# BogdanDIA/gr-dvbt

Measured on AMD Instinct MI355X. Metric: RX Msamples/s (baseband in -> TS out), higher is better.
Workload: dtype u8 (Viterbi/RS) + f32 (front end)

## Files before the change

gr_dvbt_amd/csrc/k_viterbi3.hpp:

```cpp
#pragma once
#include <hip/hip_runtime.h>
#include <stdint.h>
#include <limits.h>
#include <string.h>
#include "dvbt_tables.hpp"
#include "k_backend.hpp"

namespace dvbt {

inline VitParams make_vit_params(const Dims &d, int bsize, int chunk_bytes)
{
  VitParams v; memset(&v, 0, sizeof v);
  v.m = d.m; v.k = d.k; v.n = d.n; v.plen = d.plen; v.ntb = d.ntb; v.bsize = bsize;
  v.d_nsymbols = bsize * d.n / d.m; v.d_nbits = 2 * d.k * bsize;
  v.chunk_bytes = chunk_bytes > 0 ? chunk_bytes : 768; v.payload = d.payload; v.warm = 72;
  memcpy(v.punct, d.punct, 16); memcpy(v.prefix, d.prefix, 16);
  v.punct_mask = 0; v.prefix_nib = 0;
  for (int i = 0; i < d.plen; i++) { v.punct_mask |= (unsigned)d.punct[i] << i; v.prefix_nib |= (unsigned long long)d.prefix[i] << (4 * i); }
  v.magic_plen = ~0ull / (unsigned)d.plen + 1; v.magic_m = ~0ull / (unsigned)d.m + 1;
  for (int i = 0; i < 64; i++) v.punct_rep |= (unsigned long long)d.punct[i % d.plen] << i;
  v.magic16_plen = (65536u + (unsigned)d.plen - 1) / (unsigned)d.plen;
  return v;
}

// ... 23 lines not shown
typedef short v3pk __attribute__((ext_vector_type(2)));
__device__ __forceinline__ v3pk pk(int x) { return __builtin_bit_cast(v3pk, x); }
__device__ __forceinline__ int ipk(v3pk x) { return __builtin_bit_cast(int, x); }
__device__ __forceinline__ int pk_add(int a, int b) { return ipk(pk(a) + pk(b)); }
__device__ __forceinline__ int pk_sub(int a, int b) { return ipk(pk(a) - pk(b)); }
__device__ __forceinline__ int pk_max(int a, int b) { return ipk(__builtin_elementwise_max(pk(a), pk(b))); }
__device__ __forceinline__ int pk_min(int a, int b) { return ipk(__builtin_elementwise_min(pk(a), pk(b))); }
template <int CTRL> __device__ __forceinline__ int dppb(int v) { return __builtin_amdgcn_update_dpp(0, v, CTRL, 0xf, 0xf, true); }
__device__ __forceinline__ int vconst(int c) { int x; asm("v_mov_b32 %0, %1" : "=v"(x) : "s"(c)); return x; }
__device__ __forceinline__ int pk_max_swap(int a, int b) { int r; asm("v_pk_max_i16 %0, %1, %2 op_sel:[0,1] op_sel_hi:[1,0]" : "=v"(r) : "v"(a), "v"(b)); return r; }

struct V3Lane {
  unsigned sel[6][2];
  int bias8[6][2];
  int kc[3][2];
  int org[2];
  int arm_mid[3][2];
  int arm_b2[3][2];
  int arm_org[3][2];
};

__device__ __forceinline__ int v3_phys(int a) { const int a2 = (a >> 2) & 1; return (a & 8) | (a2 << 2) | ((a & 3) ^ (a2 ? 3 : 0)); }
__device__ __forceinline__ int v3_log(int p) { const int q = p & 7, a2 = (q >> 2) & 1; return (p & 8) | (a2 << 2) | ((q ^ (a2 ? 7 : 0)) & 3); }
__device__ __forceinline__ int v3_cell_of_z(int z) { return ((z & 2) << 4) | ((z & 1) << 4) | v3_log(z >> 2); }
__device__ __forceinline__ int v3_z_of_cell(int c) { return v3_phys(c & 15) * 4 + ((c >> 5) & 1) * 2 + ((c >> 4) & 1); }

__device__ __forceinline__ int v3_upper(int P, int r, int h, int a) { const int c = (r << 5) | (h << 4) | a; return (c >> (5 - P)) & 1; }
__device__ inline void v3_init_lane(int pl, V3Lane &L)
{
  const int a = v3_log(pl);
  for (int r = 0; r < 2; r++) {
    for (int P = 0; P < 6; P++) {
      unsigned idx[2];
      for (int h = 0; h < 2; h++) {
        const int c = (r << 5) | (h << 4) | a, i = rotl6(c, P) & 31;
        const int c0 = ((i >> 2) ^ (i >> 1) ^ i) & 1;
        const int c1 = ((i >> 4) ^ (i >> 2) ^ (i >> 1)) & 1;
        idx[h] = (unsigned)(c0 | (c1 << 1));
      }
      L.sel[P][r] = 0x0c | (idx[0] << 8) | (0x0cu << 16) | (idx[1] << 24);
      L.bias8[P][r] = (v3_upper(P, r, 0, a) << 8) | (v3_upper(P, r, 1, a) << 24);
    }
    L.org[r] = (pl * 4 + 2 * r) | ((pl * 4 + 2 * r + 1) << 16);
    for (int e = 0; e < 3; e++) {
      const int P0 = 2 * e;
      const int s0 = rotl6((r << 5) | a, P0), s1 = rotl6((r << 5) | 16 | a, P0);
      L.kc[e][r] = ((63 - s0) | ((63 - s1) << 16)) | (L.bias8[P0][r] ^ 0x01000100);
      const int b2 = ((s0 >> 4) << 6) | (((s1 >> 4) << 6) << 16);
      L.arm_mid[e][r] = (L.bias8[(P0 + 3) % 6][r] >> 2) | (L.bias8[(P0 + 4) % 6][r] >> 1) | L.bias8[(P0 + 5) % 6][r];
      L.arm_org[e][r] = L.org[r] | (L.bias8[P0][r] >> 2) | (L.bias8[P0 + 1][r] >> 1) | L.bias8[(P0 + 2) % 6][r];
      L.arm_b2[e][r] = b2 | L.bias8[P0][r];
    }
  }
}

template <int P, int ST> __device__ __forceinline__ void v3_step(int (&v)[2], unsigned W, const V3Lane &L, int (&raw)[2])
{
  int X[2], Y[2], mx[2];
  const int D0 = (int)__builtin_amdgcn_perm(0u, W, L.sel[P][0]);
  X[0] = pk_add(v[0], D0); Y[0] = pk_sub(v[0], D0);
  if (P == 0 || P == 4) { X[1] = pk_add(v[1], D0); Y[1] = pk_sub(v[1], D0); }
  else if (P == 2 || P == 3) { X[1] = pk_sub(v[1], D0); Y[1] = pk_add(v[1], D0); }
  else {
    const int D1 = (int)__builtin_amdgcn_perm(0u, W, L.sel[P][1]);
    X[1] = pk_add(v[1], D1); Y[1] = pk_sub(v[1], D1);
  }
  if (P == 0) { mx[0] = pk_max(X[0], Y[1]); mx[1] = pk_max(X[1], Y[0]); }
  else if (P == 1) { mx[0] = pk_max_swap(X[0], Y[0]); mx[1] = pk_max_swap(X[1], Y[1]); }
  else {
#pragma unroll
    for (int r = 0; r < 2; r++)
      mx[r] = pk_max(X[r], P == 2 ? dppb<DPP_ROR8>(Y[r]) : P == 3 ? dppb<DPP_HALF_MIRROR>(Y[r]) : P == 4 ? dppb<DPP_XOR2>(Y[r]) : dppb<DPP_XOR1>(Y[r]));
  }
  constexpr int PN = (P + 1) % 6;
#pragma unroll
  for (int r = 0; r < 2; r++) {
    if (ST == 0) v[r] = mx[r];
    else if (ST == 3) v[r] = (mx[r] & (int)0xfe3ffe3f) | L.arm_mid[((PN + 3) % 6) / 2][r];
    else if (ST == 1) v[r] = (mx[r] & (int)0xfe3ffe3f) | L.arm_b2[PN / 2][r];
    else if (ST == 4) v[r] = (mx[r] & (int)0xfefffeff) | L.bias8[PN][r];
    else { raw[r] = mx[r]; v[r] = (mx[r] & (int)0xfe00fe00) | L.arm_org[PN / 2][r]; }
  }
}

#if V3_EXP & 64
#define V3_YIELD() asm volatile("s_nop 3" ::: "memory")
#else
#define V3_YIELD()
#endif
template <int P0> __device__ __forceinline__ void v3_window(int (&v)[2], const unsigned (&W)[8], const V3Lane &L, int (&raw)[2])
{
  v3_step<(P0 + 0) % 6, 0>(v, W[0], L, raw); V3_YIELD(); v3_step<(P0 + 1) % 6, 0>(v, W[1], L, raw); V3_YIELD(); v3_step<(P0 + 2) % 6, 3>(v, W[2], L, raw); V3_YIELD();
  v3_step<(P0 + 3) % 6, 0>(v, W[3], L, raw); V3_YIELD(); v3_step<(P0 + 4) % 6, 0>(v, W[4], L, raw); V3_YIELD(); v3_step<(P0 + 5) % 6, 1>(v, W[5], L, raw); V3_YIELD();
  v3_step<(P0 + 6) % 6, 4>(v, W[6], L, raw); V3_YIELD(); v3_step<(P0 + 7) % 6, 2>(v, W[7], L, raw);
}

__device__ __forceinline__ int lo16(int x) { return (x << 16) >> 16; }
__device__ __forceinline__ int hi16(int x) { return x >> 16; }
template <int CTRL> __device__ __forceinline__ int max_dpp(int v) { return max(v, dppb<CTRL>(v)); }
template <int CTRL> __device__ __forceinline__ int min_dpp(int v) { return min(v, dppb<CTRL>(v)); }

template <int PE, bool RENORM> __device__ __forceinline__ int v3_window_end(int (&v)[2], const V3Lane &L)
{
  const int kp = pk_max((v[0] & (int)0xfe00fe00) | L.kc[PE / 2][0], (v[1] & (int)0xfe00fe00) | L.kc[PE / 2][1]);
  int k = max(lo16(kp), hi16(kp));
  k = max_dpp<DPP_XOR1>(k); k = max_dpp<DPP_XOR2>(k); k = max_dpp<DPP_HALF_MIRROR>(k); k = max_dpp<DPP_MIRROR>(k);
  if (RENORM) {
    const unsigned sub = (unsigned)((k & ~0x1ff) - (48 << 8));
    const int mn = (int)__builtin_amdgcn_perm(sub, sub, 0x01000100u);
    v[0] = pk_sub(v[0], mn); v[1] = pk_sub(v[1], mn);
  }
  return k;
}

struct V3Trace {
  int z[2];
  int wsh[2];
  int wlast[2];
  bool ok[2];
  long long ob[2];
};
__device__ __forceinline__ void v3_hop(V3Trace &T, const unsigned char *tab, int rowc)
{
#pragma unroll
  for (int q = 0; q < 2; q++) {
    const unsigned t = tab[T.z[q]];
    T.wsh[q] -= 256;
    T.z[q] = (T.wsh[q] & 0x3fc0) | ((int)t & ~0x3fc0);
  }
}
__device__ __forceinline__ void v3_trace_out(const V3Trace &T, const unsigned char *tab, int rowc, uint8_t *out, long long out_lo)
{
#pragma unroll
  for (int q = 0; q < 2; q++) {
    const unsigned t = tab[T.z[q]];
    const int w = T.wlast[q];
    const int sstart = rotl6(v3_cell_of_z((int)(t & 63u)), 2 * (((w % 3) + 3) % 3));
    if (T.ok[q]) out[T.ob[q] - out_lo] = (unsigned char)((sstart << 2) | (t >> 6));
  }
}

template <int V6, bool HOPS, int HOP0, int NTB> __device__ __forceinline__ void v3_fwd_window(int (&v)[2], const V3Lane &L, const unsigned *wrow, unsigned char *tab,
                                                                                           unsigned char *bests, int j0, int dd, int pl, V3Trace &T)
{
  if (HOPS && HOP0 + 2 * V6 < NTB - 1) v3_hop(T, tab, dd * 64);
  if (HOPS && HOP0 + 2 * V6 + 1 < NTB - 1) v3_hop(T, tab, dd * 64);
  const int jr = (j0 + V6) & (V3_RINGW - 1);
  unsigned W[8];
#if V3_EXP & 256
  for (int i = 0; i < 8; i++) { W[i] = (unsigned)(j0 * 0x01010101 + i * 0x00020406 + pl); asm volatile("" : "+v"(W[i])); }
#else
  {
    const uint4 *wp = reinterpret_cast<const uint4 *>(wrow + V6 * 8);
    const uint4 t0 = wp[0], t1 = wp[1];
    W[0] = t0.x; W[1] = t0.y; W[2] = t0.z; W[3] = t0.w; W[4] = t1.x; W[5] = t1.y; W[6] = t1.z; W[7] = t1.w;
  }
#endif
  constexpr int P0 = (8 * V6) % 6;
  int raw[2];
#if V3_EXP & 32
  if (V6 & 1) __builtin_amdgcn_s_setprio(1); else __builtin_amdgcn_s_setprio(0);
#endif
#if V3_EXP & 128
  __builtin_amdgcn_s_sleep(1);
#endif
  v3_window<P0>(v, W, L, raw);
  if (!(V3_EXP & 4)) *reinterpret_cast<unsigned *>(tab + (jr * 4 + dd) * 64 + pl * 4) = __builtin_amdgcn_perm((unsigned)raw[1], (unsigned)raw[0], 0x06040200u);
  if (V3_EXP & 2) { if (raw[0] == 0x12345) bests[jr] = 1; return; }
  const int s = v3_window_end<(P0 + 2) % 6, (V6 & 1) == 1>(v, L);
  bests[dd * V3_RINGW + jr] = (unsigned char)s;
}
template <bool HOPS, int HOP0, int NTB> __device__ __forceinline__ void v3_fwd_six(int (&v)[2], const V3Lane &L, const unsigned *wrow, unsigned char *tab,
                                                                                  unsigned char *bests, int j0, int dd, int pl, V3Trace &T)
{
  v3_fwd_window<0, HOPS, HOP0, NTB>(v, L, wrow, tab, bests, j0, dd, pl, T); v3_fwd_window<1, HOPS, HOP0, NTB>(v, L, wrow, tab, bests, j0, dd, pl, T);
  v3_fwd_window<2, HOPS, HOP0, NTB>(v, L, wrow, tab, bests, j0, dd, pl, T); v3_fwd_window<3, HOPS, HOP0, NTB>(v, L, wrow, tab, bests, j0, dd, pl, T);
  v3_fwd_window<4, HOPS, HOP0, NTB>(v, L, wrow, tab, bests, j0, dd, pl, T); v3_fwd_window<5, HOPS, HOP0, NTB>(v, L, wrow, tab, bests, j0, dd, pl, T);
}

#if V3_EXP & 16
__device__ unsigned long long *v3_dbg;
#endif

constexpr int V3_SLOT = 32;
constexpr int V3_CTL_CHUNKS = 0;
constexpr int V3_CTL_MISMATCH = 1;
constexpr int V3_CTL_CONFLICT = 2;
constexpr int V3_CTL_UNPROVEN = 3;
constexpr int V3_CTL_SEQ = 4;
constexpr int V3_CTL_ACC = 8;
constexpr int V3_CTL_HDR = 16;
struct V3Aux {
  int *snap;
  int *ctl;
  long long cap;
  long long grid0;
  const int *carry_in;
  int *carry_out; int carry_rel;
  int debug;
};
__device__ __forceinline__ int *v3_own(const V3Aux &ax, long long c) { return ax.snap + (3 * c) * V3_SLOT; }
__device__ __forceinline__ int *v3_pred(const V3Aux &ax, long long c) { return ax.snap + (3 * c + 1) * V3_SLOT; }
__device__ __forceinline__ int *v3_fix(const V3Aux &ax, long long c) { return ax.snap + (3 * c + 2) * V3_SLOT; }
inline size_t v3_snap_words(long long cap) { return (size_t)(cap + 2) * 3 * V3_SLOT; }
inline size_t v3_ctl_words(long long cap) { return (size_t)V3_CTL_HDR + 2 * (size_t)(cap + 2); }

struct V3Lds { unsigned char *tab; unsigned *wbuf; unsigned char *bests; const unsigned *lut; };
__device__ __forceinline__ void v3_init_lut(unsigned *lut, int lane)
{
  if (lane < 16) {
    const int k0 = (lane >> 2) & 1, k1 = (lane >> 3) & 1, t1 = (lane >> 1) & 1, t0 = lane & 1;
    const int u0 = k0 ? 1 - 2 * t1 : 0, u1 = k1 ? 1 - 2 * (k0 ? t0 : t1) : 0;
    const unsigned d0 = (unsigned)(2 * (u0 + u1)) & 0xff, d1 = (unsigned)(2 * (-u0 + u1)) & 0xff;
    const unsigned d2 = (unsigned)(2 * (u0 - u1)) & 0xff, d3 = (unsigned)(2 * (-u0 - u1)) & 0xff;
    lut[lane] = d0 | (d1 << 8) | (d2 << 16) | (d3 << 24);
  }
}

template <int NTB, int WARM, int MODE>
__device__ __forceinline__ void v3_decode(const uint8_t *__restrict__ in, uint8_t *__restrict__ out, long long total_steps, long long total_out, const VitParams &vp,
                                          long long in_base, long long out_lo, long long b0, bool dec_active, const V3Lds &S, const V3Lane &L, int (&v)[2], int (&endv)[2],
                                          int *own, int *predn, const int *inject, int *carry, int carry_rel)
{
  unsigned char *const tab = S.tab; unsigned *const wbuf = S.wbuf; unsigned char *const bests = S.bests; const unsigned *const lut = S.lut;
  unsigned *const cbits = wbuf;
  constexpr int V3_CBS = V3_BLK * 8;
  static_assert(V3_CBW <= V3_CBS, "bit stream does not fit the step-word row");
  const int lane = threadIdx.x & 63, dd = lane >> 4, pl = lane & 15;
  const int B = vp.chunk_bytes, m = vp.m;
  constexpr int ntb = NTB;
  const long long b1 = (b0 + B < total_out) ? b0 + B : total_out;
  const int warm = MODE == 2 ? 0 : WARM > 0 ? WARM : vp.warm;
  const long long w0 = b0 + 2 - warm;
  const int J = ((warm + B + ntb - 1 + V3_BLK - 1) / V3_BLK) * V3_BLK;
  const long long n_in_bytes = (total_steps * 2 / vp.plen * vp.n + vp.m - 1) / vp.m;
  const int nload = ((384 + 2 * m - 2) / m + 3 + 15) / 16;

  int ph0 = 0, bo0 = 0, off = 0; uint4 q = make_uint4(0, 0, 0, 0);
  auto stage_load = [&](int jb) {
    const long long tb = 8 * (w0 - 1) + (long long)jb * 8 - 2;
    const unsigned long long pbit = 2ull * (unsigned long long)(tb > 0 ? tb : 0);
    const unsigned long long pq = __umul64hi(pbit, vp.magic_plen);
    ph0 = (int)(pbit - pq * (unsigned)vp.plen);
    const unsigned long long rb = pq * (unsigned)vp.n + ((vp.prefix_nib >> (4 * ph0)) & 15ull);
    const unsigned long long by = __umul64hi(rb, vp.magic_m);
    const long long byte0 = (long long)by; bo0 = (int)(rb - by * (unsigned)m);
    off = (int)(((unsigned long long)(uintptr_t)in + (unsigned long long)(byte0 - in_base)) & 3ull);
    const long long src = byte0 - off + pl * 16;
    q = make_uint4(0, 0, 0, 0);
    if (dec_active && pl < nload) {
      if (src >= in_base && src + 16 <= n_in_bytes) q = *reinterpret_cast<const uint4 *>(in + (src - in_base));
      else {
        unsigned w[4] = {0, 0, 0, 0};
        for (int i = 0; i < 16; i++) {
          const long long bb = src + i;
          const unsigned bv = (bb >= in_base && bb < n_in_bytes) ? in[bb - in_base] : 0;
          w[i >> 2] |= bv << (8 * (i & 3));
        }
        q = make_uint4(w[0], w[1], w[2], w[3]);
      }
    }
  };
  auto stage_words = [&](int jb) {
    {
      const unsigned mk = (1u << m) - 1;
      auto grp = [&](unsigned d) { return ((d & mk) << (3 * m)) | (((d >> 8) & mk) << (2 * m)) | (((d >> 16) & mk) << m) | ((d >> 24) & mk); };
      const unsigned g0 = grp(q.x), g1 = grp(q.y), g2 = grp(q.z), g3 = grp(q.w);
      unsigned *cb = cbits + dd * V3_CBS;
      if (pl < nload) {
        if (m == 2) cb[pl] = (g0 << 24) | (g1 << 16) | (g2 << 8) | g3;
        else if (m == 4) { cb[2 * pl] = (g0 << 16) | g1; cb[2 * pl + 1] = (g2 << 16) | g3; }
        else { cb[3 * pl] = (g0 << 8) | (g1 >> 16); cb[3 * pl + 1] = (g1 << 16) | (g2 >> 8); cb[3 * pl + 2] = (g2 << 24) | g3; }
      }
    }
    __builtin_amdgcn_fence(__ATOMIC_SEQ_CST, "wavefront");
    constexpr int SPL = V3_BLK * 8 / 16;
    const long long tb = 8 * (w0 - 1) + (long long)jb * 8 - 2;
    const long long tbr = tb > 0 ? tb : 0;
    const int ub0 = pl * SPL;
    const long long t = tb + ub0;
    int lo = 0;
    if (t < 0) lo = (-t < SPL) ? (int)(-t) : SPL;
    const long long rem = total_steps - t;
    int hi = !dec_active ? 0 : rem <= 0 ? 0 : rem < SPL ? (int)rem : SPL;
    if (hi < lo) hi = lo;
    int x = ph0 + 2 * (int)((t + lo) - tbr);
    if (x < 0) x = 0;
    const int dq = (int)(((unsigned)x * vp.magic16_plen) >> 16);
    const int ph = x - dq * vp.plen;
    const int pos = off * m + bo0 + dq * vp.n + (int)((vp.prefix_nib >> (4 * ph)) & 15ull) - (int)((vp.prefix_nib >> (4 * ph0)) & 15ull);
    const unsigned kmask = ((unsigned)(vp.punct_rep >> ph) << (2 * lo)) & (((1u << (2 * hi)) - 1u) & ~((1u << (2 * lo)) - 1u));
    const unsigned *cb = cbits + dd * V3_CBS;
    const unsigned cw0 = cb[pos >> 5], cw1 = cb[(pos >> 5) + 1];
    unsigned win = (unsigned)(((((unsigned long long)cw0) << 32) | cw1) >> (32 - (pos & 31)));
#pragma unroll
    for (int i = 0; i < SPL; i++) {
      const unsigned k2 = (kmask >> (2 * i)) & 3u;
      const unsigned idx = (k2 << 2) | (win >> 30);
      win <<= (k2 - (k2 >> 1));
      wbuf[dd * (V3_BLK * 8) + ub0 + i] = lut[idx];
    }
    __builtin_amdgcn_fence(__ATOMIC_SEQ_CST, "wavefront");
  };
  V3Trace T;
  auto trace_init = [&](int jp) {
#pragma unroll
    for (int c = 0; c < 2; c++) {
      int jj = jp + c * 16 + pl;
      T.ob[c] = b0 + (jj - (warm + ntb - 1));
      T.ok[c] = (c * 16 + pl < V3_BLK) && dec_active && jj >= warm + ntb - 1 && T.ob[c] < b1 && (MODE != 1 || T.ob[c] >= out_lo);
      if (!T.ok[c]) jj = jp;
      const int sb = 63 - (bests[dd * V3_RINGW + (jj & (V3_RINGW - 1))] & 63);
      T.wsh[c] = ((jj << 8) & 0x3f00) | (dd * 64);
      T.z[c] = v3_z_of_cell(((sb | (sb << 6)) >> ((8 * jj + 8) % 6)) & 63) | T.wsh[c];
      T.wlast[c] = jj - (ntb - 1);
    }
  };

  stage_load(0);
  for (int jb = 0; jb < J; jb += V3_BLK) {
    if (MODE == 1 && dec_active) {
      if (jb == warm) { if (inject) { v[0] = inject[0]; v[1] = inject[1]; } own[0] = v[0]; own[1] = v[1]; }
      if (jb == warm + B) { predn[0] = v[0]; predn[1] = v[1]; }
      if (carry && jb == warm + carry_rel) { carry[0] = v[0]; carry[1] = v[1]; }
    }
    if (MODE == 2) {
      if (jb == 0 && dec_active) { own[0] = v[0]; own[1] = v[1]; }
      if (jb == B) { endv[0] = v[0]; endv[1] = v[1]; }
      if (carry && dec_active && jb == carry_rel) { carry[0] = v[0]; carry[1] = v[1]; }
    }
    if (!(V3_EXP & 8) || jb == 0) stage_words(jb);
    if (jb + V3_BLK < J && !(V3_EXP & 8)) stage_load(jb + V3_BLK);
    const bool tr = jb > 0 && !(V3_EXP & 1);
    if (tr) trace_init(jb - V3_BLK);
    const unsigned *wrow = wbuf + dd * (V3_BLK * 8);
    if (tr) {
      v3_fwd_six<true, 0, NTB>(v, L, wrow, tab, bests, jb, dd, pl, T);
      v3_fwd_six<true, 12, NTB>(v, L, wrow + 48, tab, bests, jb + 6, dd, pl, T);
      v3_trace_out(T, tab, dd * 64, out, out_lo);
    } else {
      v3_fwd_six<false, 0, NTB>(v, L, wrow, tab, bests, jb, dd, pl, T);
      v3_fwd_six<false, 0, NTB>(v, L, wrow + 48, tab, bests, jb + 6, dd, pl, T);
    }
    for (int wi = 12; wi < V3_BLK; wi += 6) v3_fwd_six<false, 0, NTB>(v, L, wrow + wi * 8, tab, bests, jb + wi, dd, pl, T);
  }
  __builtin_amdgcn_fence(__ATOMIC_SEQ_CST, "wavefront");
  trace_init(J - V3_BLK);
  for (int h = 0; h < ntb - 1; h++) v3_hop(T, tab, dd * 64);
  v3_trace_out(T, tab, dd * 64, out, out_lo);
}

#define V3_LDS_DECL(NW) \
  __shared__ __attribute__((aligned(16))) unsigned char tab_[NW][V3_RINGW * 4 * 64];    \
  __shared__ __attribute__((aligned(16))) unsigned wbuf_[NW][4 * V3_BLK * 8];           \
  __shared__ unsigned char bests_[NW][4 * V3_RINGW];                                     \
  __shared__ unsigned lut[16];

template <int NTB, int WARM = V3_WARM, int MODE = 0> __global__ __launch_bounds__(64 * V3_WGW) void viterbi3_kernel(const uint8_t *__restrict__ in, uint8_t *__restrict__ out, const RxState *st,
                                                      long long steps_fixed, VitParams vp, V3Aux ax, long long in_base, long long out_lo)
{
  V3_LDS_DECL(V3_WGW)
  const int wv = V3_WGW > 1 ? (int)(threadIdx.x >> 6) : 0;
  const V3Lds S = {tab_[wv], wbuf_[wv], bests_[wv], lut};
  const int lane = threadIdx.x & 63, dd = lane >> 4, pl = lane & 15;
  const long long total_steps = st ? st->n_vit_steps : steps_fixed;
  const long long total_out = total_steps / 8 - vp.ntb;
  const int B = vp.chunk_bytes;
  if (MODE == 1 && blockIdx.x == 0 && threadIdx.x == 0) {
    ax.ctl[V3_CTL_MISMATCH] = 0; ax.ctl[V3_CTL_CONFLICT] = 0; ax.ctl[V3_CTL_UNPROVEN] = -1; ax.ctl[V3_CTL_SEQ] = 0;
  }
  const long long grid0 = MODE == 1 ? ax.grid0 : out_lo;
  const long long chunk0 = ((long long)blockIdx.x * V3_WGW + wv) * 4;
  if (grid0 + chunk0 * B >= total_out) return;
  const long long c = chunk0 + dd, b0 = grid0 + c * B;
  const bool dec_active = b0 < total_out;
  v3_init_lut(lut, lane);
#if V3_EXP & 16
  const unsigned long long dbg_t0 = wall_clock64();
#endif
  V3Lane L; v3_init_lane(pl, L);
  int v[2] = {L.arm_org[0][0], L.arm_org[0][1]}, endv[2];
  int *own = nullptr, *predn = nullptr, *carry = nullptr; const int *inject = nullptr;
  if (MODE == 1) {
    own = v3_own(ax, c) + 2 * pl; predn = v3_pred(ax, c + 1) + 2 * pl;
    if (c == 0 && ax.carry_in) inject = ax.carry_in + 2 * pl;
    if (ax.carry_out && b0 + B >= total_out) carry = ax.carry_out + 2 * pl;
  }
  v3_decode<NTB, WARM, MODE>(in, out, total_steps, total_out, vp, in_base, out_lo, b0, dec_active, S, L, v, endv, own, predn, inject, carry, ax.carry_rel);
#if V3_EXP & 16
  if (lane == 0) {
    unsigned id, xcc;
    asm volatile("s_getreg_b32 %0, hwreg(HW_REG_HW_ID)" : "=s"(id));
    asm volatile("s_getreg_b32 %0, hwreg(HW_REG_XCC_ID)" : "=s"(xcc));
    unsigned long long *d = v3_dbg + 3 * ((long long)blockIdx.x * V3_WGW + wv);
    d[0] = (id & 0xffffu) | ((xcc & 0xfu) << 16); d[1] = dbg_t0; d[2] = wall_clock64();
  }
#endif
}

__device__ __forceinline__ long long v3_nchunks(long long total_out, long long grid0, int B) { return total_out > grid0 ? (total_out - grid0 + B - 1) / B : 0; }
__device__ __forceinline__ bool v3_slots_equal(const int *a_, const int *b_)
{
  const int4 *a = reinterpret_cast<const int4 *>(a_), *b = reinterpret_cast<const int4 *>(b_);
  bool same = true;
#pragma unroll
  for (int i = 0; i < 8; i++) { const int4 x = a[i], y = b[i]; same = same && x.x == y.x && x.y == y.y && x.z == y.z && x.w == y.w; }
  return same;
}

__global__ __launch_bounds__(256) void viterbi_check_kernel(V3Aux ax, const RxState *st, long long steps_fixed, VitParams vp, int pass)
{
  const long long total_steps = st ? st->n_vit_steps : steps_fixed;
  const long long nch = v3_nchunks(total_steps / 8 - vp.ntb, ax.grid0, vp.chunk_bytes);
  if (blockIdx.x == 0 && threadIdx.x == 0) { ax.ctl[V3_CTL_CHUNKS] = (int)(nch < INT_MAX ? nch : INT_MAX); if (pass == 1) ax.ctl[V3_CTL_UNPROVEN] = 0; }
  const long long c = (long long)blockIdx.x * 256 + threadIdx.x + 1;
  if (c >= nch || c > ax.cap) return;
  const bool same = v3_slots_equal(v3_own(ax, c), v3_pred(ax, c));
  if (pass == 0) {
    ax.ctl[V3_CTL_HDR + (ax.cap + 2) + c] = 0;
    if (!same) ax.ctl[V3_CTL_HDR + atomicAdd(ax.ctl + V3_CTL_MISMATCH, 1)] = (int)c;
  }
}
__global__ __launch_bounds__(256) void viterbi_count_kernel(V3Aux ax, const RxState *st, long long steps_fixed, VitParams vp)
{
  const long long total_steps = st ? st->n_vit_steps : steps_fixed;
  const long long nch = v3_nchunks(total_steps / 8 - vp.ntb, ax.grid0, vp.chunk_bytes);
  const long long c = (long long)blockIdx.x * 256 + threadIdx.x + 1;
  if (c >= nch || c > ax.cap) return;
  if (!v3_slots_equal(v3_own(ax, c), v3_pred(ax, c))) atomicAdd(ax.ctl + V3_CTL_UNPROVEN, 1);
}

__device__ __forceinline__ bool v3_row_equal(const int (&a)[2], const int (&b)[2], int dd)
{
  const unsigned long long ne = __ballot(a[0] != b[0] || a[1] != b[1]);
  return ((ne >> (16 * dd)) & 0xffffull) == 0;
}

template <int NTB> __device__ __forceinline__ void v3_repair_rows(const uint8_t *__restrict__ in, uint8_t *__restrict__ out, long long total_steps, const VitParams &vp, const V3Aux &ax,
                                                                  long long in_base, long long out_lo, const V3Lds &S, const V3Lane &L, long long rows, long long row0, int n)
{
  const int lane = threadIdx.x & 63, dd = lane >> 4, pl = lane & 15;
  const long long total_out = total_steps / 8 - vp.ntb;
  const int B = vp.chunk_bytes;
  const long long nch = v3_nchunks(total_out, ax.grid0, B);
  for (long long i0 = row0; i0 < n; i0 += rows) {
    const bool act = i0 + dd < n;
    const long long c = act ? ax.ctl[V3_CTL_HDR + i0 + dd] : 1;
    const long long b0 = ax.grid0 + c * B;
    int v[2], endv[2] = {0, 0};
    { const int *p = v3_pred(ax, c) + 2 * pl; v[0] = p[0]; v[1] = p[1]; }
    int *carry = (act && ax.carry_out && b0 + B >= total_out) ? ax.carry_out + 2 * pl : nullptr;
    v3_decode<NTB, 0, 2>(in, out, total_steps, total_out, vp, in_base, out_lo, b0, act && b0 < total_out, S, L, v, endv, v3_own(ax, c) + 2 * pl, nullptr, nullptr, carry, ax.carry_rel);
    int pn[2] = {endv[0], endv[1]};
    if (act && c + 1 < nch) { const int *p = v3_pred(ax, c + 1) + 2 * pl; pn[0] = p[0]; pn[1] = p[1]; }
    if (!v3_row_equal(endv, pn, dd) || ((ax.debug & 1) && act && c + 1 < nch)) {
      int *f = v3_fix(ax, c + 1) + 2 * pl; f[0] = endv[0]; f[1] = endv[1];
      if (pl == 0) { ax.ctl[V3_CTL_HDR + (ax.cap + 2) + c + 1] = 1; atomicAdd(ax.ctl + V3_CTL_CONFLICT, 1); }
    }
    __builtin_amdgcn_fence(__ATOMIC_SEQ_CST, "wavefront");
  }
}
template <int NTB> __global__ __launch_bounds__(64 * V3_WGW) void viterbi_repair_kernel(const uint8_t *__restrict__ in, uint8_t *__restrict__ out, const RxState *st,
                                                      long long steps_fixed, VitParams vp, V3Aux ax, long long in_base, long long out_lo)
{
  V3_LDS_DECL(V3_WGW)
  const int n = ax.ctl[V3_CTL_MISMATCH];
  const int wv = V3_WGW > 1 ? (int)(threadIdx.x >> 6) : 0;
  const long long rows = (long long)gridDim.x * V3_WGW * 4, row0 = ((long long)blockIdx.x * V3_WGW + wv) * 4;
  if (row0 >= n) return;
  const V3Lds S = {tab_[wv], wbuf_[wv], bests_[wv], lut};
  v3_init_lut(lut, threadIdx.x & 63);
  V3Lane L; v3_init_lane(threadIdx.x & 15, L);
  v3_repair_rows<NTB>(in, out, st ? st->n_vit_steps : steps_fixed, vp, ax, in_base, out_lo, S, L, rows, row0, n);
}

template <int NTB> __device__ __forceinline__ void v3_seq_walk(const uint8_t *__restrict__ in, uint8_t *__restrict__ out, long long total_steps, const VitParams &vp, const V3Aux &ax,
                                                               long long in_base, long long out_lo, const V3Lds &S, const V3Lane &L, int force)
{
  const int lane = threadIdx.x & 63, dd = lane >> 4, pl = lane & 15;
  if (lane == 0) { ax.ctl[V3_CTL_ACC] += ax.ctl[V3_CTL_CHUNKS]; ax.ctl[V3_CTL_ACC + 1] += ax.ctl[V3_CTL_MISMATCH]; }
  if (!force && ax.ctl[V3_CTL_CONFLICT] == 0) return;
  const long long total_out = total_steps / 8 - vp.ntb;
  const int B = vp.chunk_bytes;
  long long nch = v3_nchunks(total_out, ax.grid0, B);
  if (nch > ax.cap) nch = ax.cap;
  const int *cflag = ax.ctl + V3_CTL_HDR + (ax.cap + 2);
  int done = 0;
  long long pos = 0;
  for (;;) {
    long long cn = -1;
    for (long long c0 = pos + 1; c0 < nch && cn < 0; c0 += 64) {
      const long long c = c0 + lane;
      bool hit = false;
      if (c < nch) hit = cflag[c] != 0 || (force && !v3_slots_equal(v3_own(ax, c), v3_pred(ax, c)));
      const unsigned long long b = __ballot(hit);
      if (b) cn = c0 + __builtin_ctzll(b);
    }
    if (cn < 0) break;
    long long c = cn;
    int v[2];
    { const int *p = (cflag[c] ? v3_fix(ax, c) : v3_pred(ax, c)) + 2 * pl; v[0] = p[0]; v[1] = p[1]; }
    for (;;) {
      const long long b0 = ax.grid0 + c * B;
      const bool act = dd == 0;
      int st0[2] = {v[0], v[1]}, endv[2] = {0, 0};
      if (act) { int *p = v3_pred(ax, c) + 2 * pl; p[0] = v[0]; p[1] = v[1]; }
      int *carry = (act && ax.carry_out && b0 + B >= total_out) ? ax.carry_out + 2 * pl : nullptr;
      v3_decode<NTB, 0, 2>(in, out, total_steps, total_out, vp, in_base, out_lo, b0, act, S, L, st0, endv, v3_own(ax, c) + 2 * pl, nullptr, nullptr, carry, ax.carry_rel);
      __builtin_amdgcn_fence(__ATOMIC_SEQ_CST, "wavefront");
      done++;
      if (c + 1 >= nch) { pos = nch; break; }
      int on[2]; { const int *p = v3_own(ax, c + 1) + 2 * pl; on[0] = p[0]; on[1] = p[1]; }
      const bool eq = (__ballot(on[0] != endv[0] || on[1] != endv[1]) & 0xffffull) == 0;
      if (act) { int *p = v3_pred(ax, c + 1) + 2 * pl; p[0] = endv[0]; p[1] = endv[1]; }
      if (eq) { pos = c + 1; break; }
      c++; v[0] = endv[0]; v[1] = endv[1];
    }
  }
  if (lane == 0) { ax.ctl[V3_CTL_SEQ] = done; ax.ctl[V3_CTL_ACC + 2] += done; }
}
template <int NTB> __global__ __launch_bounds__(64) void viterbi_repair_seq_kernel(const uint8_t *__restrict__ in, uint8_t *__restrict__ out, const RxState *st,
                                                      long long steps_fixed, VitParams vp, V3Aux ax, long long in_base, long long out_lo, int force)
{
  V3_LDS_DECL(1)
  const V3Lds S = {tab_[0], wbuf_[0], bests_[0], lut};
  v3_init_lut(lut, threadIdx.x & 63);
  V3Lane L; v3_init_lane(threadIdx.x & 15, L);
  v3_seq_walk<NTB>(in, out, st ? st->n_vit_steps : steps_fixed, vp, ax, in_base, out_lo, S, L, force);
}

constexpr long long V3_FIX_SMALL = 1024;
template <int NTB> __global__ __launch_bounds__(64 * V3_WGW) void viterbi_fix_kernel(const uint8_t *__restrict__ in, uint8_t *__restrict__ out, const RxState *st,
                                                      long long steps_fixed, VitParams vp, V3Aux ax, long long in_base, long long out_lo, int force)
{
  V3_LDS_DECL(V3_WGW)
  const int wv = V3_WGW > 1 ? (int)(threadIdx.x >> 6) : 0;
  const long long total_steps = st ? st->n_vit_steps : steps_fixed;
  const long long nch = v3_nchunks(total_steps / 8 - vp.ntb, ax.grid0, vp.chunk_bytes);
  if (threadIdx.x == 0) ax.ctl[V3_CTL_CHUNKS] = (int)(nch < INT_MAX ? nch : INT_MAX);
  for (long long c = 1 + threadIdx.x; c < nch && c <= ax.cap; c += 64 * V3_WGW) {
    ax.ctl[V3_CTL_HDR + (ax.cap + 2) + c] = 0;
    if (!v3_slots_equal(v3_own(ax, c), v3_pred(ax, c))) ax.ctl[V3_CTL_HDR + atomicAdd(ax.ctl + V3_CTL_MISMATCH, 1)] = (int)c;
  }
  __threadfence(); __syncthreads();
  const int n = *(volatile int *)(ax.ctl + V3_CTL_MISMATCH);
  const V3Lds S = {tab_[wv], wbuf_[wv], bests_[wv], lut};
  v3_init_lut(lut, threadIdx.x & 63);
  V3Lane L; v3_init_lane(threadIdx.x & 15, L);
  if (!force && n > 0) v3_repair_rows<NTB>(in, out, total_steps, vp, ax, in_base, out_lo, S, L, 4 * V3_WGW, 4 * wv, n);
  __threadfence(); __syncthreads();
  if (wv == 0) v3_seq_walk<NTB>(in, out, total_steps, vp, ax, in_base, out_lo, S, L, force);
}

}
```

Before: 34700.

## Interleave traceback hops and prefetch step words in Viterbi forward windows

Restructures the Viterbi forward loop so the traceback table reads are split into read and merge halves placed between ACS steps, and the next window's step words are double-buffered (prefetched while the current window computes). It also interleaves the per-wave traceback tables into one shared LDS struct, computes stage-load byte offsets incrementally instead of with 64-bit magic divides, skips per-lane bounds clamping for interior blocks, uses a bfi for z merging, and pins lane constants in registers with empty asm. These target latency of LDS loads and scalar/integer overhead in the serial Viterbi path, at the cost of more registers and more complex index bookkeeping.

Result: faster. 36870, median of 6 (+6.3%).

```diff
diff --git a/gr_dvbt_amd/csrc/k_viterbi3.hpp b/gr_dvbt_amd/csrc/k_viterbi3.hpp
--- a/gr_dvbt_amd/csrc/k_viterbi3.hpp
+++ b/gr_dvbt_amd/csrc/k_viterbi3.hpp
@@ -99,6 +99,10 @@
       L.arm_b2[e][r] = b2 | L.bias8[P0][r];
     }
   }
+  for (int r = 0; r < 2; r++) {
+    for (int P = 0; P < 6; P++) asm("" : "+v"(L.bias8[P][r]));
+    for (int e = 0; e < 3; e++) { asm("" : "+v"(L.kc[e][r])); asm("" : "+v"(L.arm_mid[e][r])); asm("" : "+v"(L.arm_b2[e][r])); asm("" : "+v"(L.arm_org[e][r])); }
+  }
 }
 
 template <int P, int ST> __device__ __forceinline__ void v3_step(int (&v)[2], unsigned W, const V3Lane &L, int (&raw)[2])
@@ -135,12 +139,6 @@
 #else
 #define V3_YIELD()
 #endif
-template <int P0> __device__ __forceinline__ void v3_window(int (&v)[2], const unsigned (&W)[8], const V3Lane &L, int (&raw)[2])
-{
-  v3_step<(P0 + 0) % 6, 0>(v, W[0], L, raw); V3_YIELD(); v3_step<(P0 + 1) % 6, 0>(v, W[1], L, raw); V3_YIELD(); v3_step<(P0 + 2) % 6, 3>(v, W[2], L, raw); V3_YIELD();
-  v3_step<(P0 + 3) % 6, 0>(v, W[3], L, raw); V3_YIELD(); v3_step<(P0 + 4) % 6, 0>(v, W[4], L, raw); V3_YIELD(); v3_step<(P0 + 5) % 6, 1>(v, W[5], L, raw); V3_YIELD();
-  v3_step<(P0 + 6) % 6, 4>(v, W[6], L, raw); V3_YIELD(); v3_step<(P0 + 7) % 6, 2>(v, W[7], L, raw);
-}
 
 __device__ __forceinline__ int lo16(int x) { return (x << 16) >> 16; }
 __device__ __forceinline__ int hi16(int x) { return x >> 16; }
@@ -160,48 +158,57 @@
   return k;
 }
 
+template <int NW> constexpr int V3_ROW = NW * 4 * 64;
+template <int NW> constexpr int V3_RMASK = (V3_RINGW * V3_ROW<NW> - 1) & ~63;
 struct V3Trace {
   int z[2];
   int wsh[2];
-  int wlast[2];
+  int oph[2];
   bool ok[2];
-  long long ob[2];
+  int oend[2];
+  int ob[2];
 };
-__device__ __forceinline__ void v3_hop(V3Trace &T, const unsigned char *tab, int rowc)
+__device__ __forceinline__ void v3_hop_read(const V3Trace &T, const unsigned char *tab, unsigned (&t)[2])
+{
+#pragma unroll
+  for (int q = 0; q < 2; q++) t[q] = tab[T.z[q]];
+}
+template <int NW> __device__ __forceinline__ void v3_hop_merge(V3Trace &T, const unsigned (&t)[2])
+{
+#pragma unroll
+  for (int q = 0; q < 2; q++) {
+    T.wsh[q] -= V3_ROW<NW>;
+    asm("v_bfi_b32 %0, %1, %2, %3" : "=v"(T.z[q]) : "s"(V3_RMASK<NW>), "v"(T.wsh[q]), "v"(t[q]));
+  }
+}
+template <int NW> __device__ __forceinline__ void v3_hop(V3Trace &T, const unsigned char *tab) { unsigned t[2]; v3_hop_read(T, tab, t); v3_hop_merge<NW>(T, t); }
+__device__ __forceinline__ void v3_trace_out(const V3Trace &T, const unsigned char *tab, uint8_t *outb)
 {
 #pragma unroll
   for (int q = 0; q < 2; q++) {
     const unsigned t = tab[T.z[q]];
-    T.wsh[q] -= 256;
-    T.z[q] = (T.wsh[q] & 0x3fc0) | ((int)t & ~0x3fc0);
-  }
-}
-__device__ __forceinline__ void v3_trace_out(const V3Trace &T, const unsigned char *tab, int rowc, uint8_t *out, long long out_lo)
-{
-#pragma unroll
-  for (int q = 0; q < 2; q++) {
-    const unsigned t = tab[T.z[q]];
-    const int w = T.wlast[q];
-    const int sstart = rotl6(v3_cell_of_z((int)(t & 63u)), 2 * (((w % 3) + 3) % 3));
-    if (T.ok[q]) out[T.ob[q] - out_lo] = (unsigned char)((sstart << 2) | (t >> 6));
-  }
-}
-
-template <int V6, bool HOPS, int HOP0, int NTB> __device__ __forceinline__ void v3_fwd_window(int (&v)[2], const V3Lane &L, const unsigned *wrow, unsigned char *tab,
-                                                                                           unsigned char *bests, int j0, int dd, int pl, V3Trace &T)
-{
-  if (HOPS && HOP0 + 2 * V6 < NTB - 1) v3_hop(T, tab, dd * 64);
-  if (HOPS && HOP0 + 2 * V6 + 1 < NTB - 1) v3_hop(T, tab, dd * 64);
+    const int sstart = rotl6(v3_cell_of_z((int)(t & 63u)), T.oph[q]);
+    if (T.ok[q]) outb[T.ob[q]] = (unsigned char)((sstart << 2) | (t >> 6));
+  }
+}
+
+__device__ __forceinline__ void v3_load_words(const unsigned *wp_, unsigned (&W)[8])
+{
+  const uint4 *wp = reinterpret_cast<const uint4 *>(wp_);
+  const uint4 t0 = wp[0], t1 = wp[1];
+  W[0] = t0.x; W[1] = t0.y; W[2] = t0.z; W[3] = t0.w; W[4] = t1.x; W[5] = t1.y; W[6] = t1.z; W[7] = t1.w;
+}
+template <int V6, bool HOPS, int HOP0, int NTB, int NW, bool PREF> __device__ __forceinline__ void v3_fwd_window(int (&v)[2], const V3Lane &L, const unsigned *wrow, unsigned char *tab, unsigned char *tabw,
+                                                                                           unsigned char *bests, int j0, int dd, int pl, V3Trace &T, unsigned (&W)[8], unsigned (&Wn)[8])
+{
+  constexpr bool HOPA = HOPS && HOP0 + 2 * V6 < NTB - 1, HOPB = HOPS && HOP0 + 2 * V6 + 1 < NTB - 1;
+  unsigned th[2];
+  if (HOPA) v3_hop_read(T, tab, th);
   const int jr = (j0 + V6) & (V3_RINGW - 1);
-  unsigned W[8];
 #if V3_EXP & 256
   for (int i = 0; i < 8; i++) { W[i] = (unsigned)(j0 * 0x01010101 + i * 0x00020406 + pl); asm volatile("" : "+v"(W[i])); }
 #else
-  {
-    const uint4 *wp = reinterpret_cast<const uint4 *>(wrow + V6 * 8);
-    const uint4 t0 = wp[0], t1 = wp[1];
-    W[0] = t0.x; W[1] = t0.y; W[2] = t0.z; W[3] = t0.w; W[4] = t1.x; W[5] = t1.y; W[6] = t1.z; W[7] = t1.w;
-  }
+  if (PREF) v3_load_words(wrow + (V6 + 1) * 8, Wn);
 #endif
   constexpr int P0 = (8 * V6) % 6;
   int raw[2];
@@ -211,18 +218,22 @@
 #if V3_EXP & 128
   __builtin_amdgcn_s_sleep(1);
 #endif
-  v3_window<P0>(v, W, L, raw);
-  if (!(V3_EXP & 4)) *reinterpret_cast<unsigned *>(tab + (jr * 4 + dd) * 64 + pl * 4) = __builtin_amdgcn_perm((unsigned)raw[1], (unsigned)raw[0], 0x06040200u);
+  v3_step<(P0 + 0) % 6, 0>(v, W[0], L, raw); V3_YIELD(); v3_step<(P0 + 1) % 6, 0>(v, W[1], L, raw); V3_YIELD(); v3_step<(P0 + 2) % 6, 3>(v, W[2], L, raw); V3_YIELD();
+  if (HOPA) { v3_hop_merge<NW>(T, th); if (HOPB) v3_hop_read(T, tab, th); }
+  v3_step<(P0 + 3) % 6, 0>(v, W[3], L, raw); V3_YIELD(); v3_step<(P0 + 4) % 6, 0>(v, W[4], L, raw); V3_YIELD(); v3_step<(P0 + 5) % 6, 1>(v, W[5], L, raw); V3_YIELD();
+  v3_step<(P0 + 6) % 6, 4>(v, W[6], L, raw); V3_YIELD(); v3_step<(P0 + 7) % 6, 2>(v, W[7], L, raw);
+  if (HOPB) v3_hop_merge<NW>(T, th);
+  if (!(V3_EXP & 4)) *reinterpret_cast<unsigned *>(tabw + jr * V3_ROW<NW>) = __builtin_amdgcn_perm((unsigned)raw[1], (unsigned)raw[0], 0x06040200u);
   if (V3_EXP & 2) { if (raw[0] == 0x12345) bests[jr] = 1; return; }
   const int s = v3_window_end<(P0 + 2) % 6, (V6 & 1) == 1>(v, L);
   bests[dd * V3_RINGW + jr] = (unsigned char)s;
 }
-template <bool HOPS, int HOP0, int NTB> __device__ __forceinline__ void v3_fwd_six(int (&v)[2], const V3Lane &L, const unsigned *wrow, unsigned char *tab,
-                                                                                  unsigned char *bests, int j0, int dd, int pl, V3Trace &T)
-{
-  v3_fwd_window<0, HOPS, HOP0, NTB>(v, L, wrow, tab, bests, j0, dd, pl, T); v3_fwd_window<1, HOPS, HOP0, NTB>(v, L, wrow, tab, bests, j0, dd, pl, T);
-  v3_fwd_window<2, HOPS, HOP0, NTB>(v, L, wrow, tab, bests, j0, dd, pl, T); v3_fwd_window<3, HOPS, HOP0, NTB>(v, L, wrow, tab, bests, j0, dd, pl, T);
-  v3_fwd_window<4, HOPS, HOP0, NTB>(v, L, wrow, tab, bests, j0, dd, pl, T); v3_fwd_window<5, HOPS, HOP0, NTB>(v, L, wrow, tab, bests, j0, dd, pl, T);
+template <bool HOPS, int HOP0, int NTB, int NW, bool MORE> __device__ __forceinline__ void v3_fwd_six(int (&v)[2], const V3Lane &L, const unsigned *wrow, unsigned char *tab, unsigned char *tabw,
+                                                                                  unsigned char *bests, int j0, int dd, int pl, V3Trace &T, unsigned (&Wa)[8], unsigned (&Wb)[8])
+{
+  v3_fwd_window<0, HOPS, HOP0, NTB, NW, true>(v, L, wrow, tab, tabw, bests, j0, dd, pl, T, Wa, Wb); v3_fwd_window<1, HOPS, HOP0, NTB, NW, true>(v, L, wrow, tab, tabw, bests, j0, dd, pl, T, Wb, Wa);
+  v3_fwd_window<2, HOPS, HOP0, NTB, NW, true>(v, L, wrow, tab, tabw, bests, j0, dd, pl, T, Wa, Wb); v3_fwd_window<3, HOPS, HOP0, NTB, NW, true>(v, L, wrow, tab, tabw, bests, j0, dd, pl, T, Wb, Wa);
+  v3_fwd_window<4, HOPS, HOP0, NTB, NW, true>(v, L, wrow, tab, tabw, bests, j0, dd, pl, T, Wa, Wb); v3_fwd_window<5, HOPS, HOP0, NTB, NW, MORE>(v, L, wrow, tab, tabw, bests, j0, dd, pl, T, Wb, Wa);
 }
 
 #if V3_EXP & 16
@@ -252,7 +263,7 @@
 inline size_t v3_snap_words(long long cap) { return (size_t)(cap + 2) * 3 * V3_SLOT; }
 inline size_t v3_ctl_words(long long cap) { return (size_t)V3_CTL_HDR + 2 * (size_t)(cap + 2); }
 
-struct V3Lds { unsigned char *tab; unsigned *wbuf; unsigned char *bests; const unsigned *lut; };
+struct V3Lds { unsigned char *tab; unsigned *wbuf; unsigned char *bests; const unsigned *lut; int wv; };
 __device__ __forceinline__ void v3_init_lut(unsigned *lut, int lane)
 {
   if (lane < 16) {
@@ -264,7 +275,7 @@
   }
 }
 
-template <int NTB, int WARM, int MODE>
+template <int NTB, int WARM, int MODE, int NW>
 __device__ __forceinline__ void v3_decode(const uint8_t *__restrict__ in, uint8_t *__restrict__ out, long long total_steps, long long total_out, const VitParams &vp,
                                           long long in_base, long long out_lo, long long b0, bool dec_active, const V3Lds &S, const V3Lane &L, int (&v)[2], int (&endv)[2],
                                           int *own, int *predn, const int *inject, int *carry, int carry_rel)
@@ -274,6 +285,8 @@
   constexpr int V3_CBS = V3_BLK * 8;
   static_assert(V3_CBW <= V3_CBS, "bit stream does not fit the step-word row");
   const int lane = threadIdx.x & 63, dd = lane >> 4, pl = lane & 15;
+  const int rowl = S.wv * 256 + dd * 64;
+  unsigned char *const tabw = tab + rowl + pl * 4;
   const int B = vp.chunk_bytes, m = vp.m;
   constexpr int ntb = NTB;
   const long long b1 = (b0 + B < total_out) ? b0 + B : total_out;
@@ -283,15 +296,40 @@
   const long long n_in_bytes = (total_steps * 2 / vp.plen * vp.n + vp.m - 1) / vp.m;
   const int nload = ((384 + 2 * m - 2) / m + 3 + 15) / 16;
 
-  int ph0 = 0, bo0 = 0, off = 0; uint4 q = make_uint4(0, 0, 0, 0);
+  uint8_t *const outb = out + (b0 - out_lo);
+  const int ob_end = !dec_active ? INT_MIN : (int)(b1 - b0 > INT_MIN / 2 ? b1 - b0 : INT_MIN / 2);
+  const int ob_lo = MODE != 1 || out_lo <= b0 ? 0 : (int)(out_lo - b0 < INT_MAX / 2 ? out_lo - b0 : INT_MAX / 2);
+  const long long tb0 = 8 * (w0 - 1) - 2;
+  constexpr int BLKBITS = 2 * 8 * V3_BLK;
+  const int inc_q = BLKBITS / vp.plen, inc_ph = BLKBITS - inc_q * vp.plen;
+  const unsigned magic16_m = (65536u + (unsigned)m - 1) / (unsigned)m;
+
+  int u_first, u_last;
+  {
+    const long long r = total_steps - 8 * V3_BLK - tb0;
+    int first = tb0 >= 0 ? 0 : (int)((-tb0 + 7) >> 3 < J ? (-tb0 + 7) >> 3 : J), last = !dec_active || r < 0 ? -1 : (int)(r >> 3 < J ? r >> 3 : J);
+    u_first = max(max(__builtin_amdgcn_readlane(first, 0), __builtin_amdgcn_readlane(first, 16)), max(__builtin_amdgcn_readlane(first, 32), __builtin_amdgcn_readlane(first, 48)));
+    u_last = min(min(__builtin_amdgcn_readlane(last, 0), __builtin_amdgcn_readlane(last, 16)), min(__builtin_amdgcn_readlane(last, 32), __builtin_amdgcn_readlane(last, 48)));
+  }
+  int ph0 = 0, bo0 = 0, off = 0; long long byte0 = 0; uint4 q = make_uint4(0, 0, 0, 0);
   auto stage_load = [&](int jb) {
-    const long long tb = 8 * (w0 - 1) + (long long)jb * 8 - 2;
-    const unsigned long long pbit = 2ull * (unsigned long long)(tb > 0 ? tb : 0);
-    const unsigned long long pq = __umul64hi(pbit, vp.magic_plen);
-    ph0 = (int)(pbit - pq * (unsigned)vp.plen);
-    const unsigned long long rb = pq * (unsigned)vp.n + ((vp.prefix_nib >> (4 * ph0)) & 15ull);
-    const unsigned long long by = __umul64hi(rb, vp.magic_m);
-    const long long byte0 = (long long)by; bo0 = (int)(rb - by * (unsigned)m);
+    const long long tb = tb0 + (long long)jb * 8;
+    if (jb > 0 && jb - V3_BLK >= u_first) {
+      const int pf0 = (int)((vp.prefix_nib >> (4 * ph0)) & 15ull);
+      ph0 += inc_ph;
+      const int wrap = ph0 >= vp.plen ? 1 : 0;
+      ph0 -= wrap ? vp.plen : 0;
+      const int r = bo0 + (inc_q + wrap) * vp.n + (int)((vp.prefix_nib >> (4 * ph0)) & 15ull) - pf0;
+      const int dby = (int)(((unsigned)r * magic16_m) >> 16);
+      bo0 = r - dby * m; byte0 += dby;
+    } else {
+      const unsigned long long pbit = 2ull * (unsigned long long)(tb > 0 ? tb : 0);
+      const unsigned long long pq = __umul64hi(pbit, vp.magic_plen);
+      ph0 = (int)(pbit - pq * (unsigned)vp.plen);
+      const unsigned long long rb = pq * (unsigned)vp.n + ((vp.prefix_nib >> (4 * ph0)) & 15ull);
+      const unsigned long long by = __umul64hi(rb, vp.magic_m);
+      byte0 = (long long)by; bo0 = (int)(rb - by * (unsigned)m);
+    }
     off = (int)(((unsigned long long)(uintptr_t)in + (unsigned long long)(byte0 - in_base)) & 3ull);
     const long long src = byte0 - off + pl * 16;
     q = make_uint4(0, 0, 0, 0);
@@ -322,17 +360,20 @@
     }
     __builtin_amdgcn_fence(__ATOMIC_SEQ_CST, "wavefront");
     constexpr int SPL = V3_BLK * 8 / 16;
-    const long long tb = 8 * (w0 - 1) + (long long)jb * 8 - 2;
-    const long long tbr = tb > 0 ? tb : 0;
+    const long long tb = tb0 + (long long)jb * 8;
     const int ub0 = pl * SPL;
-    const long long t = tb + ub0;
-    int lo = 0;
-    if (t < 0) lo = (-t < SPL) ? (int)(-t) : SPL;
-    const long long rem = total_steps - t;
-    int hi = !dec_active ? 0 : rem <= 0 ? 0 : rem < SPL ? (int)rem : SPL;
-    if (hi < lo) hi = lo;
-    int x = ph0 + 2 * (int)((t + lo) - tbr);
-    if (x < 0) x = 0;
+    int lo = 0, hi = SPL;
+    int x = ph0 + 2 * ub0;
+    if (jb < u_first || jb > u_last) {
+      const long long tbr = tb > 0 ? tb : 0;
+      const long long t = tb + ub0;
+      if (t < 0) lo = (-t < SPL) ? (int)(-t) : SPL;
+      const long long rem = total_steps - t;
+      hi = !dec_active ? 0 : rem <= 0 ? 0 : rem < SPL ? (int)rem : SPL;
+      if (hi < lo) hi = lo;
+      x = ph0 + 2 * (int)((t + lo) - tbr);
+      if (x < 0) x = 0;
+    }
     const int dq = (int)(((unsigned)x * vp.magic16_plen) >> 16);
     const int ph = x - dq * vp.plen;
     const int pos = off * m + bo0 + dq * vp.n + (int)((vp.prefix_nib >> (4 * ph)) & 15ull) - (int)((vp.prefix_nib >> (4 * ph0)) & 15ull);
@@ -344,23 +385,25 @@
     for (int i = 0; i < SPL; i++) {
       const unsigned k2 = (kmask >> (2 * i)) & 3u;
       const unsigned idx = (k2 << 2) | (win >> 30);
-      win <<= (k2 - (k2 >> 1));
+      win <<= __popc(k2);
       wbuf[dd * (V3_BLK * 8) + ub0 + i] = lut[idx];
     }
     __builtin_amdgcn_fence(__ATOMIC_SEQ_CST, "wavefront");
   };
   V3Trace T;
+  int tph[2];
+#pragma unroll
+  for (int c = 0; c < 2; c++) { T.oend[c] = c * 16 + pl < V3_BLK ? ob_end : INT_MIN; tph[c] = 2 * ((c * 16 + pl + 1) % 3); T.oph[c] = 2 * ((c * 16 + pl + 3 * ntb - (ntb - 1)) % 3); }
+  static_assert(V3_BLK % 3 == 0, "phases per lane");
   auto trace_init = [&](int jp) {
 #pragma unroll
     for (int c = 0; c < 2; c++) {
-      int jj = jp + c * 16 + pl;
-      T.ob[c] = b0 + (jj - (warm + ntb - 1));
-      T.ok[c] = (c * 16 + pl < V3_BLK) && dec_active && jj >= warm + ntb - 1 && T.ob[c] < b1 && (MODE != 1 || T.ob[c] >= out_lo);
-      if (!T.ok[c]) jj = jp;
+      const int jj = jp + c * 16 + pl;
+      T.ob[c] = jj - (warm + ntb - 1);
+      T.ok[c] = T.ob[c] >= ob_lo && T.ob[c] < T.oend[c];
       const int sb = 63 - (bests[dd * V3_RINGW + (jj & (V3_RINGW - 1))] & 63);
-      T.wsh[c] = ((jj << 8) & 0x3f00) | (dd * 64);
-      T.z[c] = v3_z_of_cell(((sb | (sb << 6)) >> ((8 * jj + 8) % 6)) & 63) | T.wsh[c];
-      T.wlast[c] = jj - (ntb - 1);
+      T.wsh[c] = jj * V3_ROW<NW> + rowl;
+      T.z[c] = v3_z_of_cell(((sb | (sb << 6)) >> tph[c]) & 63) | (T.wsh[c] & V3_RMASK<NW>);
     }
   };
 
@@ -381,34 +424,42 @@
     const bool tr = jb > 0 && !(V3_EXP & 1);
     if (tr) trace_init(jb - V3_BLK);
     const unsigned *wrow = wbuf + dd * (V3_BLK * 8);
+    unsigned Wa[8], Wb[8];
+    v3_load_words(wrow, Wa);
     if (tr) {
-      v3_fwd_six<true, 0, NTB>(v, L, wrow, tab, bests, jb, dd, pl, T);
-      v3_fwd_six<true, 12, NTB>(v, L, wrow + 48, tab, bests, jb + 6, dd, pl, T);
-      v3_trace_out(T, tab, dd * 64, out, out_lo);
+      v3_fwd_six<true, 0, NTB, NW, true>(v, L, wrow, tab, tabw, bests, jb, dd, pl, T, Wa, Wb);
+      v3_fwd_six<true, 12, NTB, NW, true>(v, L, wrow + 48, tab, tabw, bests, jb + 6, dd, pl, T, Wa, Wb);
+      v3_trace_out(T, tab, outb);
     } else {
-      v3_fwd_six<false, 0, NTB>(v, L, wrow, tab, bests, jb, dd, pl, T);
-      v3_fwd_six<false, 0, NTB>(v, L, wrow + 48, tab, bests, jb + 6, dd, pl, T);
-    }
-    for (int wi = 12; wi < V3_BLK; wi += 6) v3_fwd_six<false, 0, NTB>(v, L, wrow + wi * 8, tab, bests, jb + wi, dd, pl, T);
+      v3_fwd_six<false, 0, NTB, NW, true>(v, L, wrow, tab, tabw, bests, jb, dd, pl, T, Wa, Wb);
+      v3_fwd_six<false, 0, NTB, NW, true>(v, L, wrow + 48, tab, tabw, bests, jb + 6, dd, pl, T, Wa, Wb);
+    }
+    static_assert(V3_BLK == 24, "the second half of the block is written out: two groups of six windows, straight-line like the first half");
+    v3_fwd_six<false, 0, NTB, NW, true>(v, L, wrow + 96, tab, tabw, bests, jb + 12, dd, pl, T, Wa, Wb);
+    v3_fwd_six<false, 0, NTB, NW, false>(v, L, wrow + 144, tab, tabw, bests, jb + 18, dd, pl, T, Wa, Wb);
   }
   __builtin_amdgcn_fence(__ATOMIC_SEQ_CST, "wavefront");
   trace_init(J - V3_BLK);
-  for (int h = 0; h < ntb - 1; h++) v3_hop(T, tab, dd * 64);
-  v3_trace_out(T, tab, dd * 64, out, out_lo);
-}
-
-#define V3_LDS_DECL(NW) \
-  __shared__ __attribute__((aligned(16))) unsigned char tab_[NW][V3_RINGW * 4 * 64];    \
-  __shared__ __attribute__((aligned(16))) unsigned wbuf_[NW][4 * V3_BLK * 8];           \
-  __shared__ unsigned char bests_[NW][4 * V3_RINGW];                                     \
-  __shared__ unsigned lut[16];
+  for (int h = 0; h < ntb - 1; h++) v3_hop<NW>(T, tab);
+  v3_trace_out(T, tab, outb);
+}
+
+template <int NW> struct V3Shared {
+  alignas(16) unsigned char tab[V3_RINGW * V3_ROW<NW>];
+  alignas(16) unsigned wbuf[NW][4 * V3_BLK * 8];
+  unsigned char bests[NW][4 * V3_RINGW];
+  unsigned lut[16];
+};
+static_assert(sizeof(V3Shared<4>) <= 81920 && V3_RMASK<4> == 0xffc0 && V3_RMASK<1> == 0x3fc0, "two four-wave workgroups per CU beside the symbol kernel's 76 KB");
+#define V3_LDS_DECL(NW) __shared__ V3Shared<NW> sh_;
+#define V3_LDS(NW, wv) V3Lds{sh_.tab, sh_.wbuf[wv], sh_.bests[wv], sh_.lut, wv}
 
 template <int NTB, int WARM = V3_WARM, int MODE = 0> __global__ __launch_bounds__(64 * V3_WGW) void viterbi3_kernel(const uint8_t *__restrict__ in, uint8_t *__restrict__ out, const RxState *st,
                                                       long long steps_fixed, VitParams vp, V3Aux ax, long long in_base, long long out_lo)
 {
   V3_LDS_DECL(V3_WGW)
   const int wv = V3_WGW > 1 ? (int)(threadIdx.x >> 6) : 0;
-  const V3Lds S = {tab_[wv], wbuf_[wv], bests_[wv], lut};
+  const V3Lds S = V3_LDS(V3_WGW, wv);
   const int lane = threadIdx.x & 63, dd = lane >> 4, pl = lane & 15;
   const long long total_steps = st ? st->n_vit_steps : steps_fixed;
   const long long total_out = total_steps / 8 - vp.ntb;
@@ -421,7 +472,7 @@
   if (grid0 + chunk0 * B >= total_out) return;
   const long long c = chunk0 + dd, b0 = grid0 + c * B;
   const bool dec_active = b0 < total_out;
-  v3_init_lut(lut, lane);
+  v3_init_lut(sh_.lut, lane);
 #if V3_EXP & 16
   const unsigned long long dbg_t0 = wall_clock64();
 #endif
@@ -433,7 +484,7 @@
     if (c == 0 && ax.carry_in) inject = ax.carry_in + 2 * pl;
     if (ax.carry_out && b0 + B >= total_out) carry = ax.carry_out + 2 * pl;
   }
-  v3_decode<NTB, WARM, MODE>(in, out, total_steps, total_out, vp, in_base, out_lo, b0, dec_active, S, L, v, endv, own, predn, inject, carry, ax.carry_rel);
+  v3_decode<NTB, WARM, MODE, V3_WGW>(in, out, total_steps, total_out, vp, in_base, out_lo, b0, dec_active, S, L, v, endv, own, predn, inject, carry, ax.carry_rel);
 #if V3_EXP & 16
   if (lane == 0) {
     unsigned id, xcc;
@@ -483,7 +534,7 @@
   return ((ne >> (16 * dd)) & 0xffffull) == 0;
 }
 
-template <int NTB> __device__ __forceinline__ void v3_repair_rows(const uint8_t *__restrict__ in, uint8_t *__restrict__ out, long long total_steps, const VitParams &vp, const V3Aux &ax,
+template <int NTB, int NW> __device__ __forceinline__ void v3_repair_rows(const uint8_t *__restrict__ in, uint8_t *__restrict__ out, long long total_steps, const VitParams &vp, const V3Aux &ax,
                                                                   long long in_base, long long out_lo, const V3Lds &S, const V3Lane &L, long long rows, long long row0, int n)
 {
   const int lane = threadIdx.x & 63, dd = lane >> 4, pl = lane & 15;
@@ -497,7 +548,7 @@
     int v[2], endv[2] = {0, 0};
     { const int *p = v3_pred(ax, c) + 2 * pl; v[0] = p[0]; v[1] = p[1]; }
     int *carry = (act && ax.carry_out && b0 + B >= total_out) ? ax.carry_out + 2 * pl : nullptr;
-    v3_decode<NTB, 0, 2>(in, out, total_steps, total_out, vp, in_base, out_lo, b0, act && b0 < total_out, S, L, v, endv, v3_own(ax, c) + 2 * pl, nullptr, nullptr, carry, ax.carry_rel);
+    v3_decode<NTB, 0, 2, NW>(in, out, total_steps, total_out, vp, in_base, out_lo, b0, act && b0 < total_out, S, L, v, endv, v3_own(ax, c) + 2 * pl, nullptr, nullptr, carry, ax.carry_rel);
     int pn[2] = {endv[0], endv[1]};
     if (act && c + 1 < nch) { const int *p = v3_pred(ax, c + 1) + 2 * pl; pn[0] = p[0]; pn[1] = p[1]; }
     if (!v3_row_equal(endv, pn, dd) || ((ax.debug & 1) && act && c + 1 < nch)) {
@@ -515,13 +566,13 @@
   const int wv = V3_WGW > 1 ? (int)(threadIdx.x >> 6) : 0;
   const long long rows = (long long)gridDim.x * V3_WGW * 4, row0 = ((long long)blockIdx.x * V3_WGW + wv) * 4;
   if (row0 >= n) return;
-  const V3Lds S = {tab_[wv], wbuf_[wv], bests_[wv], lut};
-  v3_init_lut(lut, threadIdx.x & 63);
+  const V3Lds S = V3_LDS(V3_WGW, wv);
+  v3_init_lut(sh_.lut, threadIdx.x & 63);
   V3Lane L; v3_init_lane(threadIdx.x & 15, L);
-  v3_repair_rows<NTB>(in, out, st ? st->n_vit_steps : steps_fixed, vp, ax, in_base, out_lo, S, L, rows, row0, n);
-}
-
-template <int NTB> __device__ __forceinline__ void v3_seq_walk(const uint8_t *__restrict__ in, uint8_t *__restrict__ out, long long total_steps, const VitParams &vp, const V3Aux &ax,
+  v3_repair_rows<NTB, V3_WGW>(in, out, st ? st->n_vit_steps : steps_fixed, vp, ax, in_base, out_lo, S, L, rows, row0, n);
+}
+
+template <int NTB, int NW> __device__ __forceinline__ void v3_seq_walk(const uint8_t *__restrict__ in, uint8_t *__restrict__ out, long long total_steps, const VitParams &vp, const V3Aux &ax,
                                                                long long in_base, long long out_lo, const V3Lds &S, const V3Lane &L, int force)
 {
   const int lane = threadIdx.x & 63, dd = lane >> 4, pl = lane & 15;
@@ -553,7 +604,7 @@
       int st0[2] = {v[0], v[1]}, endv[2] = {0, 0};
       if (act) { int *p = v3_pred(ax, c) + 2 * pl; p[0] = v[0]; p[1] = v[1]; }
       int *carry = (act && ax.carry_out && b0 + B >= total_out) ? ax.carry_out + 2 * pl : nullptr;
-      v3_decode<NTB, 0, 2>(in, out, total_steps, total_out, vp, in_base, out_lo, b0, act, S, L, st0, endv, v3_own(ax, c) + 2 * pl, nullptr, nullptr, carry, ax.carry_rel);
+      v3_decode<NTB, 0, 2, NW>(in, out, total_steps, total_out, vp, in_base, out_lo, b0, act, S, L, st0, endv, v3_own(ax, c) + 2 * pl, nullptr, nullptr, carry, ax.carry_rel);
       __builtin_amdgcn_fence(__ATOMIC_SEQ_CST, "wavefront");
       done++;
       if (c + 1 >= nch) { pos = nch; break; }
@@ -570,10 +621,10 @@
                                                       long long steps_fixed, VitParams vp, V3Aux ax, long long in_base, long long out_lo, int force)
 {
   V3_LDS_DECL(1)
-  const V3Lds S = {tab_[0], wbuf_[0], bests_[0], lut};
-  v3_init_lut(lut, threadIdx.x & 63);
+  const V3Lds S = V3_LDS(1, 0);
+  v3_init_lut(sh_.lut, threadIdx.x & 63);
   V3Lane L; v3_init_lane(threadIdx.x & 15, L);
-  v3_seq_walk<NTB>(in, out, st ? st->n_vit_steps : steps_fixed, vp, ax, in_base, out_lo, S, L, force);
+  v3_seq_walk<NTB, 1>(in, out, st ? st->n_vit_steps : steps_fixed, vp, ax, in_base, out_lo, S, L, force);
 }
 
 constexpr long long V3_FIX_SMALL = 1024;
@@ -591,12 +642,12 @@
   }
   __threadfence(); __syncthreads();
   const int n = *(volatile int *)(ax.ctl + V3_CTL_MISMATCH);
-  const V3Lds S = {tab_[wv], wbuf_[wv], bests_[wv], lut};
-  v3_init_lut(lut, threadIdx.x & 63);
+  const V3Lds S = V3_LDS(V3_WGW, wv);
+  v3_init_lut(sh_.lut, threadIdx.x & 63);
   V3Lane L; v3_init_lane(threadIdx.x & 15, L);
-  if (!force && n > 0) v3_repair_rows<NTB>(in, out, total_steps, vp, ax, in_base, out_lo, S, L, 4 * V3_WGW, 4 * wv, n);
+  if (!force && n > 0) v3_repair_rows<NTB, V3_WGW>(in, out, total_steps, vp, ax, in_base, out_lo, S, L, 4 * V3_WGW, 4 * wv, n);
   __threadfence(); __syncthreads();
-  if (wv == 0) v3_seq_walk<NTB>(in, out, total_steps, vp, ax, in_base, out_lo, S, L, force);
-}
-
-}
+  if (wv == 0) v3_seq_walk<NTB, V3_WGW>(in, out, total_steps, vp, ax, in_base, out_lo, S, L, force);
+}
+
+}
```
